# choderalab/pymbar

Measured on AMD Instinct MI355X. Metric: mbar_adaptive_iterations_per_sec, higher is better.
Workload: dtype f64

## Files before the change

### include/mbar_hip.h

```cpp
#ifndef MBAR_HIP_H
#define MBAR_HIP_H

#include <stdint.h>

#ifdef __cplusplus
extern "C" {
#endif

typedef struct mbar_ctx mbar_ctx;

#define MBAR_OK 0
#define MBAR_ERR_ARG (-1)
#define MBAR_ERR_HIP (-2)
#define MBAR_ERR_NODEVICE (-3)
#define MBAR_ERR_STATE (-4)
#define MBAR_ERR_COMM (-5)
#define MBAR_ERR_NUMERIC (-6)

#define MBAR_EVAL_GRAM 1u
#define MBAR_EVAL_USE_OFFSET 2u

#define MBAR_TIMER_LSE 0
#define MBAR_TIMER_GRAM 1
#define MBAR_TIMER_REDUCE 2
// ... 63 lines not shown
int mbar_gram_w(mbar_ctx* ctx, const double* f, double* gramW, double* wsum);

int mbar_ctx_create_ext(mbar_ctx** out, mbar_ctx* base, int64_t K_rows);
int mbar_ctx_rows_sub_from(mbar_ctx* dst, int64_t dst_row0, mbar_ctx* src, int64_t src_row0, int64_t nrows, const double* v_host);
int mbar_ctx_rows_rsub_from(mbar_ctx* dst, int64_t dst_row0, mbar_ctx* src, int64_t src_row0, int64_t nrows);
int mbar_ctx_rows_obs_from(mbar_ctx* dst, int64_t dst_row0, mbar_ctx* base, int64_t state_row0, int64_t obs_row0, int64_t nrows,
                           double* shift_out, const double* min_in, double* min_out);
int mbar_lognum_ext(mbar_ctx* ext, mbar_ctx* base, const double* f_base, double* lognum_ext);
int mbar_gram_w_ext(mbar_ctx* ext, mbar_ctx* base, const double* f_base, const double* f_ext, const double* gram_base, double* gramW,
                    double* wsum);

typedef struct mbar_solve_result {
    int64_t iterations;
    int64_t nr_iter;
    int64_t sci_iter;
    int32_t success;
    int32_t gram_sweeps;
    double max_delta;
    double gnorm;
    double wall_ms;
    int32_t warm_starts;
    int32_t builds;
    int32_t light_sweeps;
    int32_t reserved_;
} mbar_solve_result;

int mbar_solve_adaptive(mbar_ctx* ctx, double* f_inout, double tol, int64_t maxiter,
                        int64_t min_sc_iter, double gamma, int check_convergence,
                        double* history, int64_t history_rows, mbar_solve_result* result);
int mbar_ctx_last_solve_psum(mbar_ctx* ctx, double* psum);
int mbar_solve_sci(mbar_ctx* ctx, double* f_inout, double tol, int64_t maxiter, int check_convergence,
                   mbar_solve_result* result);

int mbar_ctx_timing(mbar_ctx* ctx, int which, double* total_ms, int64_t* launches);
int mbar_ctx_timing_reset(mbar_ctx* ctx);
int mbar_mfma_f64_peak(mbar_ctx* ctx, double* tflops);

typedef struct mbar_kde mbar_kde;
#define MBAR_KDE_GAUSSIAN 0
#define MBAR_KDE_TOPHAT 1
#define MBAR_KDE_EPANECHNIKOV 2
#define MBAR_KDE_EXPONENTIAL 3
#define MBAR_KDE_LINEAR 4
#define MBAR_KDE_COSINE 5
int mbar_kde_create(mbar_kde** out, int device, int kernel, int d, int64_t N, const double* x, double bandwidth);
void mbar_kde_destroy(mbar_kde* kde);
int mbar_kde_set_weights(mbar_kde* kde, int64_t C, const double* v);
// ... 63 lines not shown
```

### pymbar_amd/_lib.py

```python
import ctypes as C
import os

HERE = os.path.dirname(os.path.abspath(__file__))
LIB_PATH = os.environ.get("MBAR_HIP_LIBRARY") or os.path.join(HERE, "csrc", "libmbar_hip.so")

MBAR_OK = 0
EVAL_GRAM = 1
EVAL_USE_OFFSET = 2
TIMER_LSE, TIMER_GRAM, TIMER_REDUCE, TIMER_OTHER, TIMER_FUSED, TIMER_NEWTON, TIMER_COMM = 0, 1, 2, 3, 4, 5, 6


class BackendUnavailable(RuntimeError):
    """libmbar_hip.so is missing / not loadable, or there is no gfx950 device."""


class MbarHipError(RuntimeError):

    def __init__(self, code, message):
        super().__init__(f"libmbar_hip error {code}: {message}")
        self.code = code


class BarState(C.Structure):
    _fields_ = [(n, C.c_double) for n in ("DeltaF", "DeltaF_old", "DeltaF_initial", "UpperB", "LowerB", "FUpperB", "FLowerB", "FNew",
# ... 7 lines not shown


class BatchState(C.Structure):
    _fields_ = [(n, C.c_double * MBAR_BATCH_MAX_K) for n in ("f",)] + [("req", (C.c_double * MBAR_BATCH_MAX_K) * 2)] + [
        (n, C.c_double * MBAR_BATCH_MAX_K) for n in ("lognum", "psum", "Nk", "x")] + [
        (n, C.c_double) for n in ("tol", "gamma", "max_delta", "max_diff", "gnorm_sci", "gnorm_nr")] + [
        (n, C.c_int64) for n in ("K", "maxiter", "min_sc_iter", "iterations", "nr_iter", "sci_iter", "choices", "phase", "status",
                                 "success", "nreq", "gram_req", "gram_w", "newton_bad")]


class SolveResult(C.Structure):
    _fields_ = [
        ("iterations", C.c_int64),
        ("nr_iter", C.c_int64),
        ("sci_iter", C.c_int64),
        ("success", C.c_int32),
        ("gram_sweeps", C.c_int32),
        ("max_delta", C.c_double),
        ("gnorm", C.c_double),
        ("wall_ms", C.c_double),
        ("warm_starts", C.c_int32),
        ("builds", C.c_int32),
        ("light_sweeps", C.c_int32),
        ("reserved_", C.c_int32),
    ]


ALLREDUCE_FN = C.CFUNCTYPE(C.c_int, C.POINTER(C.c_double), C.c_int64, C.c_int, C.c_void_p)

_dp = C.POINTER(C.c_double)
_ip = C.POINTER(C.c_int64)
_ctx = C.c_void_p

SIGNATURES = {
    "mbar_version": (C.c_int, []),
    "mbar_last_error": (C.c_char_p, [_ctx]),
    "mbar_device_count": (C.c_int, [C.POINTER(C.c_int)]),
    "mbar_device_info": (C.c_int, [C.c_int, C.c_char_p, C.c_int, C.POINTER(C.c_int), _ip]),
    "mbar_ctx_create": (C.c_int, [C.POINTER(_ctx), C.c_int, C.c_int64, C.c_int64]),
    "mbar_ctx_destroy": (None, [_ctx]),
    "mbar_ctx_synchronize": (C.c_int, [_ctx]),
    "mbar_device_synchronize": (C.c_int, [C.c_int]),
    "mbar_cache_trim": (C.c_int, []),
    "mbar_host_digest": (C.c_int, [C.c_void_p, C.c_int64, C.c_int, C.POINTER(C.c_uint64)]),
    "mbar_host_newton_direction": (C.c_int, [_dp, _dp, C.c_int, C.c_int, _dp]),
    "mbar_ctx_set_option": (C.c_int, [_ctx, C.c_char_p, C.c_int64]),
    "mbar_ctx_upload_u": (C.c_int, [_ctx, _dp, C.c_int64, C.c_int64, C.c_int64, C.c_int64]),
# ... 191 lines not shown
```

### pymbar_amd/csrc/mbar_capi.cpp

```cpp
#include "mbar_ctx.h"

using namespace mbar;
using namespace mbar::host;

namespace mbar {
namespace host {

int fail(mbar_ctx* c, int code, const std::string& msg) {
    if (c) c->error = msg;
    g_last_error = msg;
    return code;
}
hipEvent_t get_event(mbar_ctx* c) {
    if (!c->pool.empty()) {
        hipEvent_t e = c->pool.back();
        c->pool.pop_back();
        return e;
    }
    hipEvent_t e;
    if (hipEventCreate(&e) != hipSuccess) return nullptr;
    return e;
}
void flush_timers(mbar_ctx* c) {
    for (auto& tp : c->pending) {
// ... 671 lines not shown
    if (e != hipSuccess) return fail(nullptr, MBAR_ERR_HIP, std::string("hipDeviceSynchronize: ") + hipGetErrorString(e));
    return MBAR_OK;
}

int mbar_ctx_set_option(mbar_ctx* c, const char* key, int64_t value) {
    if (!c || !key) return fail(c, MBAR_ERR_ARG, "NULL argument");
    const std::string k(key);
    if (k == "grid_blocks") c->opt_grid = value;
    else if (k == "force_generic") c->opt_force_generic = value;
    else if (k == "small_k_kernel") c->opt_small = value;
    else if (k == "wide_k_kernel") c->opt_wide = value;
    else if (k == "check_finite") c->opt_check_finite = value;
    else if (k == "timing") c->opt_timing = value;
    else if (k == "graph") c->opt_graph = value;
    else if (k == "sci_batch") c->opt_sci_batch = value < 1 ? 1 : (value > 256 ? 256 : value);
    else if (k == "device_loop") c->opt_device_loop = value;
    else if (k == "pmode") c->opt_pmode = value;
    else if (k == "fused") c->opt_fused = value;
    else if (k == "gram_quad") c->opt_quad = value;
    else if (k == "device_loop_wide") c->opt_device_loop_wide = value;
    else if (k == "pcache") c->opt_pcache = value;
    else if (k == "merge_select") c->opt_merge_select = value;
    else if (k == "light_last") c->opt_light_last = value;
    else if (k == "debug_download_p") c->opt_debug_download_p = value;
    else if (k == "direct_results") c->opt_direct_results = value;
    else if (k == "sci_merged") c->opt_sci_merged = value;
    else if (k == "host_pmode") c->opt_host_pmode = value;
    else if (k == "rect_waves") c->opt_rect_waves = value == 8 ? 8 : 4;
    else if (k == "newton_ldlt") {
        c->opt_newton_ldlt = value ? 1 : 0;
        (void)drop_graphs(c);
    }
    else if (k == "sci_pingpong") {
        c->opt_sci_pingpong = value;
        (void)drop_graphs(c);
    }
    else if (k == "small_balanced") {
        c->opt_small_balanced = value;
        (void)drop_graphs(c);
    }
    else if (k == "wide_pmode") c->opt_wide_pmode = value;
    else if (k == "quad_trim") {
        c->opt_quad_trim = value;
        c->P_valid = false;
    }
    else if (k == "adapt_batch") c->opt_adapt_batch = value < 1 ? 1 : (value > 64 ? 64 : value);
// ... 897 lines not shown
```

### pymbar_amd/csrc/mbar_ctx.h

```cpp
#pragma once
#include "../../include/mbar_hip.h"
#include "mbar_internal.h"

#include <dlfcn.h>
#include <sched.h>
#include <unistd.h>
#include <rccl/rccl.h>

#include <algorithm>
#include <chrono>
#include <condition_variable>
#include <cmath>
#include <cstdio>
#include <cstdlib>
#include <cstring>
#include <functional>
#include <limits>
#include <map>
#include <memory>
#include <mutex>
#include <string>
#include <atomic>
#include <thread>
#include <unordered_map>
// ... 244 lines not shown
    bool vec_holds_logshift = false;
    hipGraphExec_t sci_graph = nullptr;
    int64_t sci_graph_batch = 0, sci_graph_sig = 0;
    double sci_graph_tol = 0.0;
    double* ad = nullptr;
    int64_t ad_hist_cap = 0;
    int* ad_ints = nullptr;
    int* h_ctl = nullptr;
    hipGraphExec_t ad_graph = nullptr;
    int64_t ad_graph_batch = 0, ad_graph_sig = 0;
    double* P = nullptr;
    bool P_failed = false;
    double* pm_vec = nullptr;
    double* pm_ld0 = nullptr;
    double* part_g = nullptr;
    size_t part_g_doubles = 0;
    double* cwsq = nullptr;
    double* chol = nullptr;
    long long* stamps = nullptr;
    std::vector<double> last_psum;
    bool P_valid = false;
    std::vector<double> P_a0;
    int64_t opt_grid = 0, opt_force_generic = 0, opt_check_finite = 1, opt_sci_batch = 16, opt_timing = 0, opt_graph = 1, opt_small = 1, opt_wide = 1;
    int64_t opt_device_loop = 1, opt_adapt_batch = 8, opt_pmode = 1, opt_fused = 1, opt_quad = 1, opt_device_loop_wide = 1, opt_pcache = 1, opt_merge_select = 1, opt_sci_merged = 1, opt_wide_pmode = 1, opt_quad_trim = 1, opt_light_last = 1, opt_direct_results = 1, opt_debug_download_p = 0;
    int64_t opt_small_balanced = 1, opt_sci_pingpong = 1, opt_host_pmode = 2, opt_rect_waves = 8, opt_newton_ldlt = 1;

    ncclComm_t comm = nullptr;
    mbar_loopback* loop = nullptr;
    mbar_allreduce_fn host_reduce = nullptr;
    void* host_reduce_user = nullptr;
    int rank = 0, nranks = 1;
    std::vector<TimerPair> pending;
    std::vector<hipEvent_t> pool;
    double t_ms[MBAR_TIMER_COUNT] = {0, 0, 0, 0, 0};
    int64_t t_n[MBAR_TIMER_COUNT] = {0, 0, 0, 0, 0};
    std::string error;
};


namespace mbar {
namespace host {

int fail(mbar_ctx* c, int code, const std::string& msg);
#define HIPCHK(ctx, expr)                                                                        \
    do {                                                                                         \
        hipError_t _e = (expr);                                                                  \
        if (_e != hipSuccess)                                                                    \
// ... 204 lines not shown
```

### pymbar_amd/csrc/mbar_internal.h

```cpp
#pragma once
#include <hip/hip_runtime.h>
#include <stdint.h>

#include "../../include/mbar_hip.h"

namespace mbar {

constexpr int TS = 16;
constexpr int GROUPS = 4;
constexpr int MAX_FAST_K = 256;
constexpr int PANEL = 64;

inline int64_t padded_K(int64_t K) {
    if (K <= 128) return (K + 15) / 16 * 16;
    return (K + PANEL - 1) / PANEL * PANEL;
}
inline int lse_nb_for(int64_t Kp) {
    static const int nbs[] = {1, 2, 3, 4, 5, 6, 7, 8, 12, 16};
    int need = (int)(Kp / 16);
    for (int nb : nbs) if (nb >= need) return nb;
    return 0;
}

#if defined(__HIPCC__)
// ... 155 lines not shown
    double* anum;
    const double* Nk;
    const double* lnNk;
    const int* sampled;
    int m, K, Kp;
    int* ctl;
    const double* prm;
    double* state;
    double* hist;
    int64_t hist_cap;
    int pmode;
    const double* a0;
    double* ccur;
    int fused;
    double* cgram;
    int light_ok;
    long long* stamps;
    int newton_ldlt;
};
LaunchGeom psweep_geometry(int nb, int num_cu, int64_t ntiles, int64_t grid_override);
hipError_t launch_psweep(hipStream_t s, int nb, int nf, const LaunchGeom& g, const double* P, int64_t ld, int64_t N,
                         const double* cmul, const double* cw, double* rinv0, double* rinv1, double* psum_part,
                         const LoopCtl& lc = LoopCtl());
LaunchGeom fused_geometry(int nb, int num_cu, int64_t ntiles, int64_t grid_override);
hipError_t launch_fused(hipStream_t s, int nb, const LaunchGeom& g, const double* P, int64_t ld, int64_t N, const double* cmul,
                        const double* cw, const double* wsq, double* rinv_base, double* gram_part, double* psum_part,
                        const LoopCtl& lc);
LaunchGeom build_sweep_geometry(int nb, int num_cu, int64_t ntiles, int64_t grid_override);
hipError_t launch_build_sweep(hipStream_t s, int nb, const LaunchGeom& g, const double* u, int64_t ld, int64_t N,
                              const double* aden, const double* cw, double* P, double* rinv_slot, double* psum_part);
LaunchGeom build_gram_geometry(int nb, int num_cu, int64_t ntiles, int64_t grid_override);
hipError_t launch_build_gram(hipStream_t s, int nb, const LaunchGeom& g, const double* u, int64_t ld, int64_t N,
                             const double* aden, const double* wsq, bool general, double* P, double* rinv_slot, double* gram_part);

hipError_t launch_make_p(hipStream_t s, int num_cu, const double* u, int64_t ld, int64_t N, int64_t rows, const double* aden,
                         const double* logden, double* P);
hipError_t launch_fill(hipStream_t s, double* v, double value, int64_t n);
hipError_t launch_zero(hipStream_t s, void* p, size_t bytes);
hipError_t launch_sqrt_vec(hipStream_t s, double* dst, const double* src, int64_t n);
hipError_t launch_rinv_from_logden(hipStream_t s, const double* ld0, const double* ldv, const double* cw, bool weighted, int64_t N,
                                   double* out);
hipError_t launch_rinv_weighted(hipStream_t s, const double* rinv, const double* cw, int64_t N, double* out,
                                const LoopCtl& lc = LoopCtl());
hipError_t launch_newton(hipStream_t s, const AdaptArgs& a);
constexpr size_t NEWTON_CHOL_WORK = (size_t)256 * 256 + 8;
hipError_t launch_newton_chol(hipStream_t s, const AdaptArgs& a, double* work);
hipError_t launch_select(hipStream_t s, const AdaptArgs& a);
hipError_t launch_select_newton(hipStream_t s, const AdaptArgs& a);
hipError_t launch_ctl_resume(hipStream_t s, int* ctl);
// ... 435 lines not shown
```

### pymbar_amd/csrc/mbar_k_fused.hip

```cpp
#include "mbar_device.h"

namespace mbar {

template <int NB>
__host__ __device__ constexpr int fused_steps_done(int I) {
    if (I < 0) return 0;
    if (I >= NB - 2) return 2 * NB;
    if (NB < 4) return 2 * (I + 1) < 2 * NB ? 2 * (I + 1) : 2 * NB;
    const int r1 = (NB + 1) / 2 - 1;
    if (I <= r1) return 2 * (I + 1) < NB ? 2 * (I + 1) : NB;
    const int rows = NB - 2 - r1;
    return NB + (NB * (I - r1) + rows - 1) / rows;
}
template <int NB, bool WIDE>
__global__ void __launch_bounds__(256, 1)
k_fused(const double* __restrict__ P, int64_t ld, int64_t N, int64_t ntiles, const double* __restrict__ cmul,
        const double* __restrict__ cw, const double* __restrict__ wsq, double* __restrict__ rinv0,
        double* __restrict__ rinv1, double* __restrict__ gram_part, double* __restrict__ psum_part,
        const int* __restrict__ ctl, int64_t slot_stride) {
    extern __shared__ __attribute__((aligned(16))) char smem[];
    if (ctl) {
        if (ctl[CTL_DONE] != 0 || ctl[CTL_LIGHT] != 0) return;
        const int s = ctl[CTL_SLOT];
        rinv1 = rinv0 + (int64_t)((s + 2) % 3) * slot_stride;
        rinv0 = rinv0 + (int64_t)((s + 1) % 3) * slot_stride;
    }
    constexpr int ROWS = NB * 16;
    constexpr int NDMA = ROWS / 8 + 1;
    constexpr int U_BYTES = ROWS * TS * 8;
    constexpr int TILE_BYTES = U_BYTES + 1024;
    constexpr int NBLK = NB * (NB + 1) / 2;
    constexpr bool PINNED = NBLK > GRAM_AGPR_BLOCKS;
    constexpr bool ACC1 = NB < FUSED_PSUM1_FROM_GRAM_NB;
    const int lane = threadIdx.x & 63;
    const int wave = __builtin_amdgcn_readfirstlane(threadIdx.x >> 6);
    const int nwv = blockDim.x >> 6;
    const int ks = lane & 15, ns = lane >> 4;
    char* buf = smem + wave * (2 * TILE_BYTES);
    const int64_t gw = (int64_t)blockIdx.x * nwv + wave;
    const int64_t W = (int64_t)gridDim.x * nwv;
    RowIdentity rows{0};
    const StageOffsetsT<WIDE> so = make_stage_offsets<WIDE>(ld, lane);

    double acc[2][NB];
#pragma unroll
    for (int f = 0; f < 2; ++f)
#pragma unroll
        for (int I = 0; I < NB; ++I) acc[f][I] = 0.0;
    {
        double cany[NB];
#pragma unroll
        for (int I = 0; I < NB; ++I) cany[I] = fabs(cmul[16 * I + ks]) + fabs(cmul[ROWS + 16 * I + ks]);
        if constexpr (NB <= 2) rows.live = live_piece_mask<NB>(cany, 0.0);
    }
    constexpr int NSTEP = ROWS / 4;
    {
        double* ctab = reinterpret_cast<double*>(smem + nwv * (2 * TILE_BYTES));
        for (int e = threadIdx.x; e < NSTEP * 16; e += blockDim.x) ctab[e] = (e & 3) < 2 ? cmul[(e & 3) * ROWS + (e >> 2)] : 0.0;
        __syncthreads();
    }
    int apos[4];
#pragma unroll
    for (int q = 0; q < 4; ++q) apos[q] = ns * (TS * 8) + (((lane & 15) + (ns & 2) + 4 * q) & 15) * 8;
    v4d G[NBLK];
#pragma unroll
    for (int b = 0; b < NBLK; ++b) G[b] = v4d{0.0, 0.0, 0.0, 0.0};

    const int rd_base = ks * (TS * 8);
    int pos[GROUPS];
#pragma unroll
    for (int g = 0; g < GROUPS; ++g) pos[g] = ((4 * g + ns + (ks & 14)) & 15) * 8;
    const int sq = ns + 4 * ((lane >> 2) & 3);
    const int fq = lane & 3;

    const char* wsrc = reinterpret_cast<const char*>(((lane >> 3) & 1) ? wsq : cw) + (lane & 7) * 16;
    auto stage_w = [&](int64_t tile, char* dst) {
        __builtin_amdgcn_global_load_lds((const __attribute__((address_space(1))) void*)(wsrc + tile * (TS * 8)),
                                         (__attribute__((address_space(3))) void*)(dst + U_BYTES), 16, 0, 0);
    };
    auto stage = [&](int64_t tile, char* dst) {
        stage_tile<ROWS, true, 0, 1>(P, ld, tile * TS, dst, lane, so, rows);
        stage_w(tile, dst);
    };
    auto read_group = [&](const char* tb, int g, double (&x)[NB], double& wg, double& swg) {
        wg = *reinterpret_cast<const double*>(tb + U_BYTES + (4 * g + ns) * 8);
        swg = *reinterpret_cast<const double*>(tb + U_BYTES + TS * 8 + (4 * g + ns) * 8);
#pragma unroll
        for (int I = 0; I < NB; ++I) x[I] = *reinterpret_cast<const double*>(tb + I * (16 * TS * 8) + rd_base + pos[g]);
    };
    uint32_t cop_off = (uint32_t)(nwv * (2 * TILE_BYTES) + (lane >> 4) * 32 + (lane & 3) * 8);
    auto read_step = [&](const char* tb, int st, double& a, double& b) {
        a = *reinterpret_cast<const double*>(tb + st * (4 * TS * 8) + apos[st & 3]);
        b = *reinterpret_cast<const double*>(smem + cop_off + st * 128);
    };
    auto mfma4 = [&](double& d, double a, double b, bool first) {
        if constexpr (PINNED) {
            if (first)
                asm volatile("v_mfma_f64_4x4x4_4b_f64 %0, %1, %2, 0" : "=v"(d) : "v"(a), "v"(b));
            else
                asm volatile("v_mfma_f64_4x4x4_4b_f64 %0, %1, %2, %0" : "+v"(d) : "v"(a), "v"(b));
        } else {
            d = __builtin_amdgcn_mfma_f64_4x4x4f64(a, b, first ? 0.0 : d, 0, 0, 0);
        }
    };
    auto store_rinv = [&](int64_t tile, double r) {
        const int64_t n = tile * TS + sq;
        double* out = fq ? rinv1 : rinv0;
        if (n < N && fq < 2) out[n] = r;
    };
    int64_t t = gw;
    int cur = 0;
    double rcur = 0.0;
    double uv[2][NB], w[2], sw[2];
    if (t < ntiles) {
        stage(t, buf);
        if (t + W < ntiles) {
            stage(t + W, buf + TILE_BYTES);
            wait_vm<NDMA>();
        } else {
            wait_vm<0>();
        }
        double sa = 0.0, sb = 0.0;
#pragma unroll
        for (int st = 0; st < NSTEP; st += 2) {
            double a0, b0, a1, b1;
            read_step(buf, st, a0, b0);
            read_step(buf, st + 1, a1, b1);
            sa = __builtin_amdgcn_mfma_f64_4x4x4f64(a0, b0, sa, 0, 0, 0);
            sb = __builtin_amdgcn_mfma_f64_4x4x4f64(a1, b1, sb, 0, 0, 0);
        }
        rcur = recip_fast(fmax(sa + sb, 1e-300));
        store_rinv(t, rcur);
        read_group(buf, 0, uv[0], w[0], sw[0]);
    }
    for (; t < ntiles; t += W) {
        char* cbuf = buf + cur * TILE_BYTES;
        char* nbuf = buf + (cur ^ 1) * TILE_BYTES;
        const int64_t tn = t + W, tnn = t + 2 * W;
        const int64_t tstage = tnn < ntiles ? tnn : t;
        asm volatile("" : "+v"(cop_off));
        double sacc[4];
#pragma unroll
        for (int g = 0; g < GROUPS; ++g) {
            const int gc = g & 1, gn = gc ^ 1;
            if (g == 2) wait_vm<1>();
            double r0, r1;
            switch (g) {
                case 0: r0 = row16_bcast<0>(rcur); r1 = row16_bcast<1>(rcur); break;
                case 1: r0 = row16_bcast<4>(rcur); r1 = row16_bcast<5>(rcur); break;
                case 2: r0 = row16_bcast<8>(rcur); r1 = row16_bcast<9>(rcur); break;
                default: r0 = row16_bcast<12>(rcur); r1 = row16_bcast<13>(rcur); break;
            }
            const double q0 = w[gc] * r0, q1 = w[gc] * r1;
#pragma unroll
            for (int I = 0; I < NB; ++I) {
                acc[0][I] = fma(uv[gc][I], q0, acc[0][I]);
                if constexpr (ACC1) acc[1][I] = fma(uv[gc][I], q1, acc[1][I]);
                settle(acc[0][I]);
                if constexpr (ACC1) settle(acc[1][I]);
            }
            const double rin = r1 * sw[gc];
            double p[NB];
#pragma unroll
            for (int I = 0; I < NB; ++I) p[I] = uv[gc][I] * rin;
            constexpr int B1 = NB >= 4 ? NB : 2 * NB;
            double opa[B1], opb[B1];
            auto request_next = [&]() {
                if (g < GROUPS - 1) {
                    read_group(cbuf, g + 1, uv[gn], w[gn], sw[gn]);
                } else {
                    read_group(nbuf, 0, uv[gn], w[gn], sw[gn]);
                }
            };
            auto request_steps = [&]() {
                if (g >= 2) {
#pragma unroll
                    for (int q = 0; q < B1; ++q) read_step(nbuf, (g - 2) * 2 * NB + q, opa[q], opb[q]);
                }
            };
            if constexpr (!PINNED) {
                request_next();
                request_steps();
            }
            auto mfma = [&](int b, double x, double y) {
// ... 14 lines not shown
            int b = 0, nm = 0;
#pragma unroll
            for (int I = 0; I < NB; ++I) {
                if (NB == 1 && g >= 2) {
                    mfma4(sacc[2 * (g & 1)], opa[0], opb[0], true);
                    mfma4(sacc[2 * (g & 1) + 1], opa[1], opb[1], true);
                }
#pragma unroll
                for (int J = I; J < NB; ++J) {
                    mfma(b, p[I], p[J]);
                    if constexpr (PINNED) {
                        if (nm == 0 || nm == 1) {
                            __builtin_amdgcn_sched_barrier(0);
                            if (nm == 0) request_next(); else request_steps();
                            __builtin_amdgcn_sched_barrier(0);
                        }
                    }
                    if (g == GROUPS - 1) {
#pragma unroll
                        for (int j = nm * NDMA / NM; j < (nm + 1) * NDMA / NM; ++j) {
                            if constexpr (PINNED) __builtin_amdgcn_sched_barrier(0);
                            if (j < ROWS / 8)
                                stage_piece<true>(P + rows(8 * j) * ld + rows.cols(j, tstage * TS), so.off[j & 1], cbuf + j * 1024, lane);
                            else
                                stage_w(tstage, cbuf);
                            if constexpr (PINNED) __builtin_amdgcn_sched_barrier(0);
                        }
                    }
                    ++b;
                    ++nm;
                }
                if (g >= 2 && NB > 1 && I < NB - 1) {
#pragma unroll
                    for (int q = fused_steps_done<NB>(I - 1); q < fused_steps_done<NB>(I); ++q)
                        mfma4(sacc[q & 3], opa[q % B1], opb[q % B1], g == 2 && q < 4);
                    if (B1 < 2 * NB && fused_steps_done<NB>(I - 1) < B1 && fused_steps_done<NB>(I) >= B1) {
#pragma unroll
                        for (int q = 0; q < B1; ++q) read_step(nbuf, (g - 2) * 2 * NB + B1 + q, opa[q], opb[q]);
                    }
                }
            }
            if constexpr (PINNED) __builtin_amdgcn_sched_barrier(0);
        }
        if constexpr (PINNED)
            asm volatile("s_nop 7\n\ts_nop 7" : "+v"(sacc[0]), "+v"(sacc[1]), "+v"(sacc[2]), "+v"(sacc[3]));
        rcur = recip_fast(fmax((sacc[0] + sacc[1]) + (sacc[2] + sacc[3]), 1e-300));
        store_rinv(tn, rcur);
// ... 10 lines not shown
            if (lane < 16) psum_part[(gw * 2 + f) * ROWS + 16 * I + lane] = v;
        }
    }
    {
        int b = 0;
#pragma unroll
        for (int I = 0; I < NB; ++I)
#pragma unroll
            for (int J = I; J < NB; ++J, ++b) {
#pragma unroll
                for (int r = 0; r < 4; ++r) {
#if defined(MBAR_GRAM_STORE_NT)
                    __builtin_nontemporal_store(G[b][r], &gram_part[((gw * NBLK + b) * 4 + r) * 64 + lane]);
#else
                    gram_part[((gw * NBLK + b) * 4 + r) * 64 + lane] = G[b][r];
#endif
                }
            }
    }
}



LaunchGeom fused_geometry(int nb, int num_cu, int64_t ntiles, int64_t grid_override) {
    LaunchGeom g;
    g.waves = 4;
    g.variant = 1;
    if (nb > 8) {
        g.variant = 6;
        g.lds_bytes = (size_t)2 * ((size_t)nb * 16 * TS * 8 + 4 * 1024) + 1024;
        int64_t capq = grid_override > 0 ? grid_override : num_cu;
        int64_t wantq = ntiles < 1 ? 1 : ntiles;
        g.blocks = (int)(wantq < capq ? wantq : capq);
        g.nwaves = g.blocks;
        g.psum_records = g.nwaves;
        return g;
    }
    const size_t tile = (size_t)nb * 16 * TS * 8 + 1024;
    g.lds_bytes = (size_t)4 * 2 * tile + (size_t)nb * 512;
    int64_t want = (ntiles + 3) / 4;
    int64_t cap = num_cu;
    if (nb <= 5) {
        static const int occ[6] = {1, 4, 4, 3, 2, 2};
        const int by_lds = blocks_per_cu_for(g.lds_bytes);
        cap = (int64_t)num_cu * (by_lds < occ[nb] ? by_lds : occ[nb]);
        int64_t by_work = (ntiles + 127) / 128;
        if (by_work < num_cu) by_work = num_cu;
        if (cap > by_work) cap = by_work;
    }
    if (grid_override > 0) cap = grid_override;
    if (want < 1) want = 1;
    g.blocks = (int)(want < cap ? want : cap);
    g.nwaves = g.blocks * 4;
    g.psum_records = g.nwaves;
    return g;
}
template <int NB>
static hipError_t launch_fused_nb(hipStream_t s, const LaunchGeom& g, const double* P, int64_t ld, int64_t N, const double* cmul,
                                  const double* cw, const double* wsq, double* rinv0, double* gp, double* pp, const LoopCtl& lc) {
    auto go = [&](auto kern) -> hipError_t {
        if (g.lds_bytes > 64 * 1024) {
            hipError_t e = hipFuncSetAttribute(reinterpret_cast<const void*>(kern),
                                               hipFuncAttributeMaxDynamicSharedMemorySize, (int)g.lds_bytes);
            if (e != hipSuccess) return e;
        }
        const int64_t ntiles = (N + TS - 1) / TS;
        double* r1 = nullptr;
        if (lc.ev_start && lc.ev_stop)
            hipExtLaunchKernelGGL(kern, dim3(g.blocks), dim3(256), g.lds_bytes, s, lc.ev_start, lc.ev_stop, 0, P, ld, N, ntiles, cmul,
                                  cw, wsq, rinv0, r1, gp, pp, lc.ctl, lc.slot_stride);
        else
            hipLaunchKernelGGL(kern, dim3(g.blocks), dim3(256), g.lds_bytes, s, P, ld, N, ntiles, cmul, cw, wsq, rinv0, r1, gp, pp,
                               lc.ctl, lc.slot_stride);
        return hipGetLastError();
    };
    return stage_offsets_wide(ld) ? go(k_fused<NB, true>) : go(k_fused<NB, false>);
}
hipError_t launch_fused(hipStream_t s, int nb, const LaunchGeom& g, const double* P, int64_t ld, int64_t N, const double* cmul,
                        const double* cw, const double* wsq, double* rinv_base, double* gram_part, double* psum_part,
                        const LoopCtl& lc) {
    if (!lc.ctl) return hipErrorInvalidValue;
    if (nb == 12 || nb == 16) return launch_fused_quad(s, nb, g, P, ld, N, cmul, cw, wsq, rinv_base, gram_part, psum_part, lc);
    switch (nb) {
#define MBAR_CASE(NB_) \
    case NB_: return launch_fused_nb<NB_>(s, g, P, ld, N, cmul, cw, wsq, rinv_base, gram_part, psum_part, lc);
        MBAR_CASE(1) MBAR_CASE(2) MBAR_CASE(3) MBAR_CASE(4) MBAR_CASE(5) MBAR_CASE(6) MBAR_CASE(7) MBAR_CASE(8)
#undef MBAR_CASE
        default: return hipErrorInvalidValue;
    }
}

}
```

### pymbar_amd/csrc/mbar_loops.cpp

```cpp
#include "mbar_ctx.h"

using namespace mbar;
using namespace mbar::host;

namespace mbar {
namespace host {

int adaptive_host_loop(mbar_ctx* c, std::vector<double>& f, double tol, int64_t maxiter, int64_t min_sc_iter, double gamma,
                       int check_convergence, double* history, int64_t history_rows, mbar_solve_result& res,
                       std::vector<double>& psum, double& max_delta) {
    const int64_t K = c->K;
    const int m = (int)c->sampled.size();
    const int first = c->sampled[0];
    std::vector<double> f_old(K), cand(2 * (size_t)K), psum2(2 * (size_t)K);
    std::vector<double> H((size_t)m * m), g(m), x;
    std::vector<int> pos((size_t)K, -1);
    for (int i = 0; i < m; ++i) pos[(size_t)c->sampled[i]] = i;
    psum.assign(K, 0.0);
    int cur = 0;
    int rc = eval_core(c, f.data(), 1, 0, c->logden[cur], nullptr, psum.data(), nullptr, nullptr);
    if (rc) return rc;
    bool done = false;
    const GramPlan plan = plan_for(c);
    const bool dbg = std::getenv("MBAR_DEBUG_TIMING") != nullptr;
// ... 294 lines not shown
                c->P_failed = true;
                pmode = false;
            } else if (launch_zero(c->stream, c->P, (size_t)Kp * c->ld * sizeof(double)) != hipSuccess) {
                arc = fail(c, MBAR_ERR_HIP, "zero fill of P failed");
            }
        }
    }
    {
        bool p_ok = pmode;
        int rc = agree_all_ok(c, p_ok);
        if (rc) return rc;
        if (pmode && !p_ok) {
            pmode = false;
            c->error = "resident probability matrix does not fit on every rank: classic sweeps";
        }
    }
    if (!arc && pmode && !c->pm_vec && cache_malloc((void**)&c->pm_vec, (size_t)3 * Kp * sizeof(double)) != hipSuccess)
        arc = fail(c, MBAR_ERR_HIP, "allocation of the P-mode vectors failed");
    const bool fused = pmode && c->opt_fused;
    bool light = fused && check_convergence && c->opt_light_last != 0 &&
                 (c->opt_light_last >= 2 || (nb >= 5 && (double)Kp * (double)c->N >= 5.0e7));
    LaunchGeom gg = wide ? gram_quad_geometry(nb, c->num_cu, ntiles, c->opt_grid)
                         : gram_geometry(nb * 16, true, c->num_cu, ntiles, c->opt_grid);
    LaunchGeom gl = fused ? fused_geometry(nb, c->num_cu, ntiles, c->opt_grid)
                    : pmode ? psweep_geometry(nb, c->num_cu, ntiles, c->opt_grid)
                            : lse_geometry(nb, 2, c->num_cu, ntiles, c->opt_grid, lse_variant_for(c));
    if (wide) gg.live_blocks = gl.live_blocks = quad_live_blocks(c);
    if (fused) {
        gg.blocks = gl.blocks;
        gg.nwaves = gl.nwaves;
    }
    LaunchGeom gp = psweep_geometry(wide ? 8 : nb, c->num_cu, ntiles, 0);
    if (light && !wide && gl.nwaves % gp.waves != 0) light = false;
    if (light && !wide) {
        gp.blocks = gl.nwaves / gp.waves;
        gp.nwaves = gp.psum_records = gl.nwaves;
    }
    {
        bool l_ok = light;
        int rcl = agree_all_ok(c, l_ok);
        if (rcl) return rcl;
        light = light && l_ok;
    }
    const LaunchGeom gb = fused ? build_gram_geometry(nb, c->num_cu, ntiles, c->opt_grid)
                                : build_sweep_geometry(nb, c->num_cu, ntiles, c->opt_grid);
    const size_t rec_g = (size_t)nb * (nb + 1) / 2 * 256;
    const size_t rec_l = (size_t)2 * Kp;
// ... 28 lines not shown
    for (int64_t k = 0; warm && k < Kp; ++k) {
        const bool live = !std::isinf(an0[k]), was = !std::isinf(c->P_a0[k]);
        if (live != was) warm = false;
        else if (live) {
            const double d = an0[k] - c->P_a0[k];
            if (!(std::fabs(d) < 200.0)) warm = false;
            cm0[k] = std::exp(d);
        }
    }
    rc = agree_all_ok(c, warm);
    if (rc) return rc;
    if (!pmode) {
        rc = eval_core(c, f.data(), 1, 0, c->logden[0], nullptr, psum.data(), nullptr, nullptr);
        if (rc) return rc;
    } else if (warm) {
        std::vector<int> z((size_t)CTL_WORDS, 0);
        HIPCHK(c, hipMemcpyAsync(c->ad_ints, z.data(), z.size() * sizeof(int), hipMemcpyHostToDevice, c->stream));
        std::copy(cm0.begin(), cm0.end(), c->hstage);
        std::copy(cm0.begin(), cm0.end(), c->hstage + Kp);
        HIPCHK(c, hipMemcpyAsync(d_aden(c), c->hstage, (size_t)2 * Kp * sizeof(double), hipMemcpyHostToDevice, c->stream));
        HIPCHK(c, hipMemsetAsync(c->red, 0, off_gram * sizeof(double), c->stream));
        {
            ScopedTimer t(c, MBAR_TIMER_OTHER);
            HIPCHK(c, launch_fused(c->stream, nb, gl, c->P, c->ld, c->N, d_aden(c), c->cw, c->weighted ? c->cwsq : c->cw, c->logden[0],
                                   c->part_g, c->part, lc_slot));
        }
        HIPCHK(c, launch_reduce2(c->stream, c->part, (int64_t)rec_l, c->part_g, (int64_t)rec_g, gl.nwaves, c->scratch, c->red,
                                 c->red + off_gram));
        rc = allreduce_dev(c, c->red, (int64_t)(off_gram + rec_g), 0);
        if (rc) return rc;
        HIPCHK(c, hipMemcpyAsync(c->hred, c->red, (size_t)Kp * sizeof(double), hipMemcpyDeviceToHost, c->stream));
        rc = sync_stream(c);
        if (rc) return rc;
        for (int64_t k = 0; k < K; ++k) psum[k] = c->hred[k] * cm0[k];
        res.warm_starts += 1;
    } else if (wide) {
        c->P_valid = false;
        rc = eval_core(c, f.data(), 1, 0, c->logden[1], nullptr, psum.data(), nullptr, nullptr);
        if (rc) return rc;
        if (fused && !c->weighted) {
            ScopedTimer t(c, MBAR_TIMER_OTHER);
            HIPCHK(c, launch_gram_quad(c->stream, nb, gg, c->u, c->ld, c->N, d_aden(c), c->logden[1], c->part_g, LoopCtl(), c->P));
            HIPCHK(c, launch_reduce(c->stream, c->part_g, gg.nwaves, (int64_t)rec_g, c->scratch, c->red + off_gram));
            rc = allreduce_dev(c, c->red + off_gram, (int64_t)rec_g, 0);
            if (rc) return rc;
            HIPCHK(c, launch_fill(c->stream, c->logden[0], 1.0, c->ld));
        } else {
            ScopedTimer t(c, MBAR_TIMER_OTHER);
// ... 185 lines not shown
        const bool split = timed && c->opt_timing == 3;
        if (!fused) {
            int r2 = enqueue_gram(timed);
            if (r2) return r2;
        }
        {
            Section sec(c, split && (wide || !merged || need_newton), MBAR_TIMER_NEWTON);
            if (wide)
                HIPCHK(c, launch_newton_chol(c->stream, q, c->chol));
            else if (!merged || need_newton)
                HIPCHK(c, launch_newton(c->stream, q));
        }
        need_newton = false;
        double* psum_part = c->part;
        double* obj_part = c->part + (size_t)gl.nwaves * rec_l;
        {
            TimerPair tp{nullptr, nullptr, fused ? MBAR_TIMER_FUSED : MBAR_TIMER_LSE};
            if (timed) { tp.a = get_event(c); tp.b = get_event(c); }
            const bool ext = tp.a && tp.b && c->opt_timing == 2;
            LoopCtl lcb = lc_slot;
            if (ext) { lcb.ev_start = tp.a; lcb.ev_stop = tp.b; }
            if (tp.a && tp.b && !ext) (void)hipEventRecord(tp.a, c->stream);
            if (fused) {
                HIPCHK(c, launch_fused(c->stream, nb, gl, c->P, c->ld, c->N, d_aden(c), c->cw, c->weighted ? c->cwsq : c->cw,
                                       c->logden[0], gram_part, psum_part, lcb));
                if (light && !wide) {
                    LoopCtl lcl = lc_slot;
                    lcl.light_only = true;
                    HIPCHK(c, launch_psweep(c->stream, nb, 2, gp, c->P, c->ld, c->N, d_aden(c), c->cw, c->logden[0], nullptr, psum_part, lcl));
                }
            } else if (pmode)
                HIPCHK(c, launch_psweep(c->stream, nb, 2, gl, c->P, c->ld, c->N, d_aden(c), c->cw, c->logden[0], nullptr, psum_part,
                                        lcb));
            else
                HIPCHK(c, launch_lse(c->stream, nb, 2, gl, c->u, c->ld, c->N, d_aden(c), c->cw, c->logden[0], nullptr,
                                     nullptr, psum_part, obj_part, lcb));
            if (tp.a && tp.b && !ext) (void)hipEventRecord(tp.b, c->stream);
            if (tp.a && tp.b) c->pending.push_back(tp);
        }
        int64_t ar_count = (int64_t)(rec_l + 2);
        {
            Section sec(c, split, MBAR_TIMER_REDUCE);
            if (fused) {
                HIPCHK(c, launch_reduce2(c->stream, psum_part, (int64_t)rec_l, gram_part, (int64_t)rec_g, gl.nwaves, c->scratch, c->red,
                                         c->red + off_gram));
                ar_count = (int64_t)(off_gram + rec_g);
            } else if (pmode) {
// ... 114 lines not shown
        HIPCHK(c, hipStreamSynchronize(c->stream));
        for (int64_t k = 0; k < K; ++k) {
            f[k] = h[ad_off_f(c) + k];
            psum[k] = h[ad_off_psum(c) + k];
        }
        if (it > res.iterations) max_delta = h[ad_off_state(c)];
    }
    if (q.stamps) {
        std::vector<long long> st(65 * 16);
        HIPCHK(c, hipMemcpy(st.data(), c->stamps, st.size() * sizeof(long long), hipMemcpyDeviceToHost));
        for (int i = 0; i < 64; ++i) {
            const long long* p = st.data() + 16 * i;
            if (!p[0] || !p[5]) continue;
            std::fprintf(stderr, "[mbar] k_select_newton launch %d (shader clocks): select %lld, set-up %lld, elimination %lld, solution %lld, candidates %lld, total %lld; of the elimination: pivot loops %lld, exchange + trailing update %lld; of the selection: inputs %lld, Gram staged %lld, matrix-vector product %lld, sums %lld, maxima %lld\n",
                         i, p[1] - p[0], p[2] - p[1], p[3] - p[2], p[4] - p[3], p[5] - p[4], p[5] - p[0], p[6], p[7], p[8] - p[0], p[9] - p[8], p[10] - p[9],
                         p[11] - p[10], p[12] - p[11]);
        }
    }
    res.iterations = it;
    res.sci_iter = c->h_ctl[CTL_SCI];
    res.nr_iter = c->h_ctl[CTL_NR];
    res.gram_sweeps += fused ? gram_sweeps : (int32_t)(it - it_start);
    res.light_sweeps += c->h_ctl[CTL_LIGHTS];
    if (handed_back) {
        c->P_valid = false;
        static const char* why[] = {"", "the Newton system is not positive definite", "a candidate is too far from the point the sweeps are anchored at",
                                    "a candidate is not finite"};
        const int r = c->h_ctl[CTL_REASON];
        c->error = std::string("device-resident adaptive loop handed back to the host loop: ") + why[(r >= 1 && r <= 3) ? r : 0];
    }
    return MBAR_OK;
}


}
}

extern "C" {

int mbar_solve_adaptive(mbar_ctx* c, double* f_inout, double tol, int64_t maxiter, int64_t min_sc_iter, double gamma,
                        int check_convergence, double* history, int64_t history_rows, mbar_solve_result* result) {
    if (c && c->ext_base) return fail(c, MBAR_ERR_STATE, "mbar_solve_adaptive: an extension context holds rows only (mbar_lognum_ext / mbar_gram_w_ext sweep them)");
    if (!c || !f_inout) return fail(c, MBAR_ERR_ARG, "NULL argument");
    if (!c->have_Nk) return fail(c, MBAR_ERR_STATE, "mbar_ctx_set_Nk has not been called");
    HIPCHK(c, hipSetDevice(c->device));
    const double t0 = now_ms();
// ... 308 lines not shown
```

Baseline: 294.9.

## Add unit-weight specialization of fused sweep kernel skipping weight staging

Result: faster. 301.0 (median of 6 runs) (+2.1%).

```diff
diff --git a/include/mbar_hip.h b/include/mbar_hip.h
--- a/include/mbar_hip.h
+++ b/include/mbar_hip.h
@@ -109,7 +109,7 @@
     int32_t warm_starts;
     int32_t builds;
     int32_t light_sweeps;
-    int32_t reserved_;
+    int32_t fused_unit;
 } mbar_solve_result;
 
 int mbar_solve_adaptive(mbar_ctx* ctx, double* f_inout, double tol, int64_t maxiter,
diff --git a/pymbar_amd/_lib.py b/pymbar_amd/_lib.py
--- a/pymbar_amd/_lib.py
+++ b/pymbar_amd/_lib.py
@@ -53,7 +53,7 @@
         ("warm_starts", C.c_int32),
         ("builds", C.c_int32),
         ("light_sweeps", C.c_int32),
-        ("reserved_", C.c_int32),
+        ("fused_unit", C.c_int32),
     ]
 
 
diff --git a/pymbar_amd/csrc/mbar_capi.cpp b/pymbar_amd/csrc/mbar_capi.cpp
--- a/pymbar_amd/csrc/mbar_capi.cpp
+++ b/pymbar_amd/csrc/mbar_capi.cpp
@@ -717,6 +717,10 @@
     else if (k == "pcache") c->opt_pcache = value;
     else if (k == "merge_select") c->opt_merge_select = value;
     else if (k == "light_last") c->opt_light_last = value;
+    else if (k == "fused_general") {
+        c->opt_fused_general = value ? 1 : 0;
+        (void)drop_graphs(c);
+    }
     else if (k == "debug_download_p") c->opt_debug_download_p = value;
     else if (k == "direct_results") c->opt_direct_results = value;
     else if (k == "sci_merged") c->opt_sci_merged = value;
diff --git a/pymbar_amd/csrc/mbar_ctx.h b/pymbar_amd/csrc/mbar_ctx.h
--- a/pymbar_amd/csrc/mbar_ctx.h
+++ b/pymbar_amd/csrc/mbar_ctx.h
@@ -290,7 +290,7 @@
     bool P_valid = false;
     std::vector<double> P_a0;
     int64_t opt_grid = 0, opt_force_generic = 0, opt_check_finite = 1, opt_sci_batch = 16, opt_timing = 0, opt_graph = 1, opt_small = 1, opt_wide = 1;
-    int64_t opt_device_loop = 1, opt_adapt_batch = 8, opt_pmode = 1, opt_fused = 1, opt_quad = 1, opt_device_loop_wide = 1, opt_pcache = 1, opt_merge_select = 1, opt_sci_merged = 1, opt_wide_pmode = 1, opt_quad_trim = 1, opt_light_last = 1, opt_direct_results = 1, opt_debug_download_p = 0;
+    int64_t opt_device_loop = 1, opt_adapt_batch = 8, opt_pmode = 1, opt_fused = 1, opt_quad = 1, opt_device_loop_wide = 1, opt_pcache = 1, opt_merge_select = 1, opt_sci_merged = 1, opt_wide_pmode = 1, opt_quad_trim = 1, opt_light_last = 1, opt_direct_results = 1, opt_debug_download_p = 0, opt_fused_general = 0;
     int64_t opt_small_balanced = 1, opt_sci_pingpong = 1, opt_host_pmode = 2, opt_rect_waves = 8, opt_newton_ldlt = 1;
 
     ncclComm_t comm = nullptr;
diff --git a/pymbar_amd/csrc/mbar_internal.h b/pymbar_amd/csrc/mbar_internal.h
--- a/pymbar_amd/csrc/mbar_internal.h
+++ b/pymbar_amd/csrc/mbar_internal.h
@@ -201,9 +201,9 @@
 hipError_t launch_psweep(hipStream_t s, int nb, int nf, const LaunchGeom& g, const double* P, int64_t ld, int64_t N,
                          const double* cmul, const double* cw, double* rinv0, double* rinv1, double* psum_part,
                          const LoopCtl& lc = LoopCtl());
-LaunchGeom fused_geometry(int nb, int num_cu, int64_t ntiles, int64_t grid_override);
+LaunchGeom fused_geometry(int nb, int num_cu, int64_t ntiles, int64_t grid_override, bool unit = false);
 hipError_t launch_fused(hipStream_t s, int nb, const LaunchGeom& g, const double* P, int64_t ld, int64_t N, const double* cmul,
-                        const double* cw, const double* wsq, double* rinv_base, double* gram_part, double* psum_part,
+                        const double* cw, const double* wsq, bool unit, double* rinv_base, double* gram_part, double* psum_part,
                         const LoopCtl& lc);
 LaunchGeom build_sweep_geometry(int nb, int num_cu, int64_t ntiles, int64_t grid_override);
 hipError_t launch_build_sweep(hipStream_t s, int nb, const LaunchGeom& g, const double* u, int64_t ld, int64_t N,
diff --git a/pymbar_amd/csrc/mbar_k_fused.hip b/pymbar_amd/csrc/mbar_k_fused.hip
--- a/pymbar_amd/csrc/mbar_k_fused.hip
+++ b/pymbar_amd/csrc/mbar_k_fused.hip
@@ -12,7 +12,7 @@
     const int rows = NB - 2 - r1;
     return NB + (NB * (I - r1) + rows - 1) / rows;
 }
-template <int NB, bool WIDE>
+template <int NB, bool WIDE, bool UNIT>
 __global__ void __launch_bounds__(256, 1)
 k_fused(const double* __restrict__ P, int64_t ld, int64_t N, int64_t ntiles, const double* __restrict__ cmul,
         const double* __restrict__ cw, const double* __restrict__ wsq, double* __restrict__ rinv0,
@@ -26,9 +26,9 @@
         rinv0 = rinv0 + (int64_t)((s + 1) % 3) * slot_stride;
     }
     constexpr int ROWS = NB * 16;
-    constexpr int NDMA = ROWS / 8 + 1;
+    constexpr int NDMA = ROWS / 8 + (UNIT ? 0 : 1);
     constexpr int U_BYTES = ROWS * TS * 8;
-    constexpr int TILE_BYTES = U_BYTES + 1024;
+    constexpr int TILE_BYTES = U_BYTES + (UNIT ? 0 : 1024);
     constexpr int NBLK = NB * (NB + 1) / 2;
     constexpr bool PINNED = NBLK > GRAM_AGPR_BLOCKS;
     constexpr bool ACC1 = NB < FUSED_PSUM1_FROM_GRAM_NB;
@@ -54,7 +54,15 @@
         if constexpr (NB <= 2) rows.live = live_piece_mask<NB>(cany, 0.0);
     }
     constexpr int NSTEP = ROWS / 4;
-    {
+    double cb[UNIT ? NSTEP : 1];
+    if constexpr (UNIT) {
+#pragma unroll
+        for (int st = 0; st < NSTEP; ++st) {
+            const double cv = cmul[(lane & 1) * ROWS + 4 * st + (lane >> 4)];
+            cb[st] = (lane & 3) < 2 ? cv : 0.0;
+            asm volatile("" : "+v"(cb[st]));
+        }
+    } else {
         double* ctab = reinterpret_cast<double*>(smem + nwv * (2 * TILE_BYTES));
         for (int e = threadIdx.x; e < NSTEP * 16; e += blockDim.x) ctab[e] = (e & 3) < 2 ? cmul[(e & 3) * ROWS + (e >> 2)] : 0.0;
         __syncthreads();
@@ -80,18 +88,21 @@
     };
     auto stage = [&](int64_t tile, char* dst) {
         stage_tile<ROWS, true, 0, 1>(P, ld, tile * TS, dst, lane, so, rows);
-        stage_w(tile, dst);
+        if constexpr (!UNIT) stage_w(tile, dst);
     };
     auto read_group = [&](const char* tb, int g, double (&x)[NB], double& wg, double& swg) {
-        wg = *reinterpret_cast<const double*>(tb + U_BYTES + (4 * g + ns) * 8);
-        swg = *reinterpret_cast<const double*>(tb + U_BYTES + TS * 8 + (4 * g + ns) * 8);
+        if constexpr (!UNIT) {
+            wg = *reinterpret_cast<const double*>(tb + U_BYTES + (4 * g + ns) * 8);
+            swg = *reinterpret_cast<const double*>(tb + U_BYTES + TS * 8 + (4 * g + ns) * 8);
+        }
 #pragma unroll
         for (int I = 0; I < NB; ++I) x[I] = *reinterpret_cast<const double*>(tb + I * (16 * TS * 8) + rd_base + pos[g]);
     };
     uint32_t cop_off = (uint32_t)(nwv * (2 * TILE_BYTES) + (lane >> 4) * 32 + (lane & 3) * 8);
     auto read_step = [&](const char* tb, int st, double& a, double& b) {
         a = *reinterpret_cast<const double*>(tb + st * (4 * TS * 8) + apos[st & 3]);
-        b = *reinterpret_cast<const double*>(smem + cop_off + st * 128);
+        if constexpr (UNIT) b = cb[st];
+        else b = *reinterpret_cast<const double*>(smem + cop_off + st * 128);
     };
     auto mfma4 = [&](double& d, double a, double b, bool first) {
         if constexpr (PINNED) {
@@ -103,9 +114,10 @@
             d = __builtin_amdgcn_mfma_f64_4x4x4f64(a, b, first ? 0.0 : d, 0, 0, 0);
         }
     };
-    auto store_rinv = [&](int64_t tile, double r) {
+    auto store_rinv = [&](int64_t tile, double& r) {
         const int64_t n = tile * TS + sq;
         double* out = fq ? rinv1 : rinv0;
+        if constexpr (UNIT) r = n < N ? r : 0.0;
         if (n < N && fq < 2) out[n] = r;
     };
     int64_t t = gw;
@@ -138,7 +150,7 @@
         char* nbuf = buf + (cur ^ 1) * TILE_BYTES;
         const int64_t tn = t + W, tnn = t + 2 * W;
         const int64_t tstage = tnn < ntiles ? tnn : t;
-        asm volatile("" : "+v"(cop_off));
+        if constexpr (!UNIT) asm volatile("" : "+v"(cop_off));
         double sacc[4];
 #pragma unroll
         for (int g = 0; g < GROUPS; ++g) {
@@ -151,7 +163,7 @@
                 case 2: r0 = row16_bcast<8>(rcur); r1 = row16_bcast<9>(rcur); break;
                 default: r0 = row16_bcast<12>(rcur); r1 = row16_bcast<13>(rcur); break;
             }
-            const double q0 = w[gc] * r0, q1 = w[gc] * r1;
+            const double q0 = UNIT ? r0 : w[gc] * r0, q1 = UNIT ? r1 : w[gc] * r1;
 #pragma unroll
             for (int I = 0; I < NB; ++I) {
                 acc[0][I] = fma(uv[gc][I], q0, acc[0][I]);
@@ -159,7 +171,7 @@
                 settle(acc[0][I]);
                 if constexpr (ACC1) settle(acc[1][I]);
             }
-            const double rin = r1 * sw[gc];
+            const double rin = UNIT ? r1 : r1 * sw[gc];
             double p[NB];
 #pragma unroll
             for (int I = 0; I < NB; ++I) p[I] = uv[gc][I] * rin;
@@ -220,7 +232,7 @@
                             if constexpr (PINNED) __builtin_amdgcn_sched_barrier(0);
                             if (j < ROWS / 8)
                                 stage_piece<true>(P + rows(8 * j) * ld + rows.cols(j, tstage * TS), so.off[j & 1], cbuf + j * 1024, lane);
-                            else
+                            else if constexpr (!UNIT)
                                 stage_w(tstage, cbuf);
                             if constexpr (PINNED) __builtin_amdgcn_sched_barrier(0);
                         }
@@ -277,7 +289,7 @@
 
 
 
-LaunchGeom fused_geometry(int nb, int num_cu, int64_t ntiles, int64_t grid_override) {
+LaunchGeom fused_geometry(int nb, int num_cu, int64_t ntiles, int64_t grid_override, bool unit) {
     LaunchGeom g;
     g.waves = 4;
     g.variant = 1;
@@ -292,12 +304,13 @@
         return g;
     }
     const size_t tile = (size_t)nb * 16 * TS * 8 + 1024;
-    g.lds_bytes = (size_t)4 * 2 * tile + (size_t)nb * 512;
+    const size_t lds_general = (size_t)4 * 2 * tile + (size_t)nb * 512;
+    g.lds_bytes = unit ? (size_t)4 * 2 * (tile - 1024) : lds_general;
     int64_t want = (ntiles + 3) / 4;
     int64_t cap = num_cu;
     if (nb <= 5) {
         static const int occ[6] = {1, 4, 4, 3, 2, 2};
-        const int by_lds = blocks_per_cu_for(g.lds_bytes);
+        const int by_lds = blocks_per_cu_for(lds_general);
         cap = (int64_t)num_cu * (by_lds < occ[nb] ? by_lds : occ[nb]);
         int64_t by_work = (ntiles + 127) / 128;
         if (by_work < num_cu) by_work = num_cu;
@@ -312,7 +325,7 @@
 }
 template <int NB>
 static hipError_t launch_fused_nb(hipStream_t s, const LaunchGeom& g, const double* P, int64_t ld, int64_t N, const double* cmul,
-                                  const double* cw, const double* wsq, double* rinv0, double* gp, double* pp, const LoopCtl& lc) {
+                                  const double* cw, const double* wsq, bool unit, double* rinv0, double* gp, double* pp, const LoopCtl& lc) {
     auto go = [&](auto kern) -> hipError_t {
         if (g.lds_bytes > 64 * 1024) {
             hipError_t e = hipFuncSetAttribute(reinterpret_cast<const void*>(kern),
@@ -329,16 +342,17 @@
                                lc.ctl, lc.slot_stride);
         return hipGetLastError();
     };
-    return stage_offsets_wide(ld) ? go(k_fused<NB, true>) : go(k_fused<NB, false>);
+    if (unit) return stage_offsets_wide(ld) ? go(k_fused<NB, true, true>) : go(k_fused<NB, false, true>);
+    return stage_offsets_wide(ld) ? go(k_fused<NB, true, false>) : go(k_fused<NB, false, false>);
 }
 hipError_t launch_fused(hipStream_t s, int nb, const LaunchGeom& g, const double* P, int64_t ld, int64_t N, const double* cmul,
-                        const double* cw, const double* wsq, double* rinv_base, double* gram_part, double* psum_part,
+                        const double* cw, const double* wsq, bool unit, double* rinv_base, double* gram_part, double* psum_part,
                         const LoopCtl& lc) {
     if (!lc.ctl) return hipErrorInvalidValue;
     if (nb == 12 || nb == 16) return launch_fused_quad(s, nb, g, P, ld, N, cmul, cw, wsq, rinv_base, gram_part, psum_part, lc);
     switch (nb) {
 #define MBAR_CASE(NB_) \
-    case NB_: return launch_fused_nb<NB_>(s, g, P, ld, N, cmul, cw, wsq, rinv_base, gram_part, psum_part, lc);
+    case NB_: return launch_fused_nb<NB_>(s, g, P, ld, N, cmul, cw, wsq, unit, rinv_base, gram_part, psum_part, lc);
         MBAR_CASE(1) MBAR_CASE(2) MBAR_CASE(3) MBAR_CASE(4) MBAR_CASE(5) MBAR_CASE(6) MBAR_CASE(7) MBAR_CASE(8)
 #undef MBAR_CASE
         default: return hipErrorInvalidValue;
diff --git a/pymbar_amd/csrc/mbar_loops.cpp b/pymbar_amd/csrc/mbar_loops.cpp
--- a/pymbar_amd/csrc/mbar_loops.cpp
+++ b/pymbar_amd/csrc/mbar_loops.cpp
@@ -340,7 +340,8 @@
                  (c->opt_light_last >= 2 || (nb >= 5 && (double)Kp * (double)c->N >= 5.0e7));
     LaunchGeom gg = wide ? gram_quad_geometry(nb, c->num_cu, ntiles, c->opt_grid)
                          : gram_geometry(nb * 16, true, c->num_cu, ntiles, c->opt_grid);
-    LaunchGeom gl = fused ? fused_geometry(nb, c->num_cu, ntiles, c->opt_grid)
+    const bool unit = !c->weighted && !c->opt_fused_general;
+    LaunchGeom gl = fused ? fused_geometry(nb, c->num_cu, ntiles, c->opt_grid, unit)
                     : pmode ? psweep_geometry(nb, c->num_cu, ntiles, c->opt_grid)
                             : lse_geometry(nb, 2, c->num_cu, ntiles, c->opt_grid, lse_variant_for(c));
     if (wide) gg.live_blocks = gl.live_blocks = quad_live_blocks(c);
@@ -415,8 +416,8 @@
         HIPCHK(c, hipMemsetAsync(c->red, 0, off_gram * sizeof(double), c->stream));
         {
             ScopedTimer t(c, MBAR_TIMER_OTHER);
-            HIPCHK(c, launch_fused(c->stream, nb, gl, c->P, c->ld, c->N, d_aden(c), c->cw, c->weighted ? c->cwsq : c->cw, c->logden[0],
-                                   c->part_g, c->part, lc_slot));
+            HIPCHK(c, launch_fused(c->stream, nb, gl, c->P, c->ld, c->N, d_aden(c), c->cw, c->weighted ? c->cwsq : c->cw, unit,
+                                   c->logden[0], c->part_g, c->part, lc_slot));
         }
         HIPCHK(c, launch_reduce2(c->stream, c->part, (int64_t)rec_l, c->part_g, (int64_t)rec_g, gl.nwaves, c->scratch, c->red,
                                  c->red + off_gram));
@@ -648,7 +649,7 @@
             if (ext) { lcb.ev_start = tp.a; lcb.ev_stop = tp.b; }
             if (tp.a && tp.b && !ext) (void)hipEventRecord(tp.a, c->stream);
             if (fused) {
-                HIPCHK(c, launch_fused(c->stream, nb, gl, c->P, c->ld, c->N, d_aden(c), c->cw, c->weighted ? c->cwsq : c->cw,
+                HIPCHK(c, launch_fused(c->stream, nb, gl, c->P, c->ld, c->N, d_aden(c), c->cw, c->weighted ? c->cwsq : c->cw, unit,
                                        c->logden[0], gram_part, psum_part, lcb));
                 if (light && !wide) {
                     LoopCtl lcl = lc_slot;
@@ -809,6 +810,7 @@
     res.nr_iter = c->h_ctl[CTL_NR];
     res.gram_sweeps += fused ? gram_sweeps : (int32_t)(it - it_start);
     res.light_sweeps += c->h_ctl[CTL_LIGHTS];
+    if (fused && !wide && unit) res.fused_unit += 1;
     if (handed_back) {
         c->P_valid = false;
         static const char* why[] = {"", "the Newton system is not positive definite", "a candidate is too far from the point the sweeps are anchored at",
```
